# researchmm/MM-Diffusion

Hardware: AMD Instinct MI355X
Metric: denoising steps/sec (video+audio pair), 16x64x64 / 25600 (higher is better)
Workload: dtype bf16; 1 GPU; BASELINE configs[1]: Landscape base model (133.68M params), DDPM p_sample, timestep_respacing=250, per-GPU batch 4, 16x3x64x64 video + 1x25600 audio; global_batch=4, parallelism=batch-sharded x1, no in-loop collective, weights=key-seeded synthetic (mm_diffusion.synth), graph_replay=True, batch_lanes=2, finite=True, ranks_seen=1

## Files before the change

### include/mmd.h

```cpp
#ifndef MMD_H
#define MMD_H
#include <stdint.h>
#ifdef __cplusplus
extern "C" {
#endif

#define MMD_F32 0
#define MMD_BF16 1
#define MMD_OK 0
#define MMD_ERR_ARG (-1)
#define MMD_ERR_LAUNCH (-2)
#define MMD_ERR_UNSUPPORTED (-3)

int mmd_version(void);
const char* mmd_last_error(void);
int mmd_debug_install_crash_handler(void);

int mmd_graph_begin(void* stream);
int mmd_graph_end(void* stream, void** exec_out);
int mmd_graph_launch(void* exec, void* stream);
int mmd_graph_destroy(void* exec);
int mmd_stream_create(void** stream_out);
int mmd_stream_sync(void* stream);
int mmd_stream_destroy(void* stream);
// ... 65 lines not shown
int mmd_tattn_block(const void* X, int64_t ldx, const void* A, int64_t lda, void* MID, int64_t ldm, const void* Wf,
                    const float* bias_pre, const float* bias_qkv, const float* bias_proj, const float* gamma, const float* beta,
                    float eps, void* Y, int64_t ldy, int N, int F, int HW, int C, int heads, float* stats, int64_t stats_ld,
                    void* stream);

int64_t mmd_tconv_weight_bytes(int Cin, int Cout);
int mmd_tconv_pack(const void* W, void* out, int Cin, int Cout, void* stream);
int mmd_tconv(const void* X, int64_t ldx, const void* Wf, const float* bias, void* Y, int64_t ldy, int N, int F, int HW, int Cin,
              int Cout, float* stats, int64_t stats_ld, void* stream);

int mmd_aconv(const void* X, int64_t ldx, const void* W, const float* bias, const float* ga, const float* gb, int act, void* Y, int64_t ldy,
              int M, int L, int Cin, int Cout, int dil, float* stats, int64_t stats_ld, void* stream);

int mmd_attn_fwd(int dtype, const void* Q, int64_t ldq, int q_off, const void* KV, int64_t ldkv, int k_off, int v_off, void* O,
                 int64_t ldo, int heads, int ch, int nb, int G, int64_t q_rows_per_batch, int q_per_group,
                 int64_t k_rows_per_batch, int k_per_group, int win, const int* shift_dev, int impl, void* stream);
int mmd_attn_small_fwd(int dtype, const void* QKV, int64_t ld, void* O, int64_t ldo, int C, int heads, int S, int Tn, int inner,
                       int64_t outer_stride, int64_t inner_stride, int64_t tstride, void* stream);

int mmd_resample(int dtype, const void* x, int64_t ldx, void* y, int64_t ldy, int C, int NF, int H, int W, int fh, int fw,
                 int mode, float scale, void* stream);
int mmd_resample_stats(const void* x, int64_t ldx, void* y, int64_t ldy, int C, int NF, int H, int W, int fh, int fw, int mode,
                       float* stats, int64_t stats_ld, void* stream);
int mmd_copy2d(const void* x, int64_t ldx_bytes, void* y, int64_t ldy_bytes, int64_t rows, int64_t row_bytes, void* stream);

int mmd_stem_conv(int dtype, const float* x, const float* w, const float* bias, void* y, int64_t ldy, int N, int F, int Cin,
                  int H, int W, int Cout, int ntaps, const int* taps, void* stream);
int mmd_head_conv(int dtype, const void* x, int64_t ldx, const float* w, const float* bias, float* y, int N, int F, int Cin,
                  int H, int W, int Co, int ntaps, const int* taps, void* stream);
int64_t mmd_head_gemm_weight_bytes(int Cin);
int64_t mmd_head_gemm_workspace_bytes(int64_t M, int ntaps, int Co);
int mmd_head_gemm(const void* x, int64_t ldx, int64_t M, int Cin, const float* gn_a, const float* gn_b, int S, int64_t gn_rows, int act,
                  const void* wimg, float* P, int NO, void* stream);
int mmd_head_gather(const float* P, const float* bias, float* y, int N, int F, int H, int W, int Co, int ntaps, const int* taps,
                    void* stream);

int mmd_ddpm_update(const float* x, const float* model_out, const float* noise, float* out, float* x0_out, float* mean_out,
                    float* logvar_out, const float* tables, const int64_t* t, int T, int N, int F, int C, int HW, int flags,
                    void* stream);
int mmd_q_sample(const float* x0, const float* eps, float* out, const float* tab2, const int64_t* t, int T, int N,
                 int64_t per_sample, void* stream);

int64_t mmd_loss_workspace_bytes(int N);
int mmd_loss_terms(const float* x0, const float* xt, const float* model_out, const float* target, const float* tables,
                   const int64_t* t, int T, int N, int F, int C, int HW, int flags, float vb_scale, float* mse_out, float* vb_out,
                   void* workspace, void* stream);
// ... 104 lines not shown
```

### mm-diffusion_amd/csrc/mmd_misc.hip

```cpp
#include "mmd_common.h"

__global__ __launch_bounds__(256) void temb_kernel(const void* __restrict__ t, int t_kind, int dim, const float* __restrict__ W0,
                                                   const float* __restrict__ b0, const float* __restrict__ W2,
                                                   const float* __restrict__ b2, float* __restrict__ out_silu,
                                                   float* __restrict__ out_raw) {
  extern __shared__ float sm[];
  float* e = sm;
  float* h = sm + dim;
  const int n = blockIdx.x, tid = threadIdx.x;
  float tv;
  if (t_kind == 0) tv = (float)((const int64_t*)t)[n];
  else if (t_kind == 1) tv = (float)((const int32_t*)t)[n];
  else tv = ((const float*)t)[n];
  const int half = dim / 2;
  for (int i = tid; i < dim; i += 256) {
    float v = 0.f;
    if (i < 2 * half) {
      const int k = i < half ? i : i - half;
      const float f = expf(-logf(10000.f) * (float)k / (float)half);
      const float a = tv * f;
      v = i < half ? cosf(a) : sinf(a);
    }
    e[i] = v;
  }
  __syncthreads();
  for (int j = tid; j < dim; j += 256) {
    float a = b0[j];
    for (int k = 0; k < dim; ++k) a += W0[j * dim + k] * e[k];
    h[j] = silu_f(a);
  }
  __syncthreads();
  for (int j = tid; j < dim; j += 256) {
    float a = b2[j];
    for (int k = 0; k < dim; ++k) a += W2[j * dim + k] * h[k];
    if (out_raw) out_raw[n * dim + j] = a;
    out_silu[n * dim + j] = silu_f(a);
  }
}

__global__ __launch_bounds__(256) void linear_kernel(const float* __restrict__ x, const float* __restrict__ W,
                                                     const float* __restrict__ b, float* __restrict__ y, int N, int K, int J) {
  const int lane = threadIdx.x & 63;
  const int j = blockIdx.x * 4 + (threadIdx.x >> 6);
  if (j >= J) return;
  for (int n0 = 0; n0 < N; n0 += 8) {
    float acc[8];
#pragma unroll
    for (int i = 0; i < 8; ++i) acc[i] = 0.f;
    for (int k = lane; k < K; k += 64) {
      const float w = W[(int64_t)j * K + k];
#pragma unroll
      for (int i = 0; i < 8; ++i)
        if (n0 + i < N) acc[i] += w * x[(int64_t)(n0 + i) * K + k];
    }
#pragma unroll
    for (int i = 0; i < 8; ++i) {
      const float s = wave_sum(acc[i]);
      if (lane == 0 && n0 + i < N) y[(int64_t)(n0 + i) * J + j] = s + (b ? b[j] : 0.f);
    }
  }
}

template <typename T>
__global__ __launch_bounds__(256) void resample_kernel(const char* __restrict__ x, int64_t ldx, char* __restrict__ y, int64_t ldy,
                                                       int C, int NF, int H, int W, int fh, int fw, int mode, float scale) {
  constexpr int EPV = Elt<T>::EPV;
  constexpr int ES = 16 / EPV;
  const int CV = C / EPV;
  const int Ho = mode == 0 ? H / fh : H * fh, Wo = mode == 0 ? W / fw : W * fw;
  const int64_t total = (int64_t)NF * Ho * Wo * CV;
  for (int64_t i = (int64_t)blockIdx.x * 256 + threadIdx.x; i < total; i += (int64_t)gridDim.x * 256) {
    const int cv = (int)(i % CV);
    const int64_t orow = i / CV;
    const int wo = (int)(orow % Wo), ho = (int)((orow / Wo) % Ho);
    const int64_t nf = orow / ((int64_t)Wo * Ho);
    float acc[EPV];
    if (mode == 0) {
#pragma unroll
      for (int e = 0; e < EPV; ++e) acc[e] = 0.f;
      for (int a = 0; a < fh; ++a)
        for (int b = 0; b < fw; ++b) {
          const int64_t irow = (nf * H + ho * fh + a) * W + wo * fw + b;
          float f[EPV];
          Elt<T>::unpack(*(const u32x4*)(x + (irow * ldx + (int64_t)cv * EPV) * ES), f);
#pragma unroll
          for (int e = 0; e < EPV; ++e) acc[e] += f[e];
        }
      const float inv = scale / (float)(fh * fw);
#pragma unroll
      for (int e = 0; e < EPV; ++e) acc[e] *= inv;
      *(u32x4*)(y + (orow * ldy + (int64_t)cv * EPV) * ES) = Elt<T>::pack(acc);
    } else {
      const int64_t irow = (nf * H + ho / fh) * W + wo / fw;
      u32x4 v = *(const u32x4*)(x + (irow * ldx + (int64_t)cv * EPV) * ES);
      if (scale != 1.f) {
        Elt<T>::unpack(v, acc);
#pragma unroll
        for (int e = 0; e < EPV; ++e) acc[e] *= scale;
        v = Elt<T>::pack(acc);
      }
      *(u32x4*)(y + (orow * ldy + (int64_t)cv * EPV) * ES) = v;
    }
  }
}

__global__ __launch_bounds__(256) void resample_stats_kernel(const char* __restrict__ x, int64_t ldx, char* __restrict__ y, int64_t ldy, int C,
                                                             int NF, int H, int W, int fh, int fw, int mode, float* __restrict__ stats,
                                                             int64_t stats_ld, int nrec, int lcvp) {
  __shared__ float sPart[256 * 4];
  const int tid = threadIdx.x, CV = C >> 3;
  const int cv = tid & ((1 << lcvp) - 1), rg = tid >> lcvp, rgn = 256 >> lcvp;
  const int Ho = mode == 0 ? H / fh : H * fh, Wo = mode == 0 ? W / fw : W * fw;
  const float inv = 1.f / (float)(fh * fw);
  for (int rec = blockIdx.x; rec < nrec; rec += gridDim.x) {
    float s0 = 0.f, s1 = 0.f, q0 = 0.f, q1 = 0.f;
    if (cv < CV) {
#pragma unroll 4
      for (int r = rg; r < 64; r += rgn) {
        const int orow = rec * 64 + r;
        const int wo = orow % Wo, t = orow / Wo, ho = t % Ho, nf = t / Ho;
        u32x4 v;
        if (mode == 0) {
          float acc[8];
#pragma unroll
          for (int e = 0; e < 8; ++e) acc[e] = 0.f;
          for (int a = 0; a < fh; ++a)
            for (int b = 0; b < fw; ++b) {
              const int64_t irow = ((int64_t)nf * H + ho * fh + a) * W + wo * fw + b;
              float f[8];
              Elt<__bf16>::unpack(*(const u32x4*)(x + (irow * ldx + (int64_t)cv * 8) * 2), f);
#pragma unroll
              for (int e = 0; e < 8; ++e) acc[e] += f[e];
            }
#pragma unroll
          for (int e = 0; e < 8; ++e) acc[e] *= inv;
          v = Elt<__bf16>::pack(acc);
        } else {
          const int64_t irow = ((int64_t)nf * H + ho / fh) * W + wo / fw;
          v = *(const u32x4*)(x + (irow * ldx + (int64_t)cv * 8) * 2);
        }
        *(u32x4*)(y + ((int64_t)orow * ldy + (int64_t)cv * 8) * 2) = v;
        float f[8];
        Elt<__bf16>::unpack(v, f);
#pragma unroll
        for (int j = 0; j < 4; ++j) {
          s0 += f[j];
          s1 += f[4 + j];
          q0 += f[j] * f[j];
          q1 += f[4 + j] * f[4 + j];
        }
      }
    }
    *(f32x4*)(sPart + tid * 4) = f32x4{s0, s1, q0, q1};
    __syncthreads();
    if (rg == 0 && cv < CV) {
      for (int g = 1; g < rgn; ++g) {
        const f32x4 o = *(const f32x4*)(sPart + ((g << lcvp) + cv) * 4);
        s0 += o[0];
        s1 += o[1];
        q0 += o[2];
        q1 += o[3];
      }
      *(f32x4*)(stats + ((int64_t)rec * stats_ld + 2 * cv) * 2) = f32x4{s0, q0, s1, q1};
    }
    __syncthreads();
  }
}

__global__ __launch_bounds__(256) void copy2d_kernel(const char* __restrict__ x, int64_t ldx_b, char* __restrict__ y, int64_t ldy_b,
                                                     int64_t rows, int vecs) {
  const int64_t total = rows * vecs;
  for (int64_t i = (int64_t)blockIdx.x * 256 + threadIdx.x; i < total; i += (int64_t)gridDim.x * 256) {
    const int64_t r = i / vecs;
    const int v = (int)(i % vecs);
    *(u32x4*)(y + r * ldy_b + (int64_t)v * 16) = *(const u32x4*)(x + r * ldx_b + (int64_t)v * 16);
  }
}

extern "C" int mmd_temb_fwd(const void* t, int t_kind, int N, int dim, const float* W0, const float* b0, const float* W2,
                            const float* b2, float* out_silu, float* out_raw, void* stream) {
  MMD_REQUIRE(t && W0 && b0 && W2 && b2 && out_silu && N > 0 && dim > 0 && dim <= 4096, "temb_fwd: bad argument");
  MMD_REQUIRE(t_kind >= 0 && t_kind <= 2, "temb_fwd: t_kind must be 0 (int64), 1 (int32) or 2 (float32)");
  return mmd_launch<temb_kernel>("temb", dim3(N), dim3(256), 2 * dim * sizeof(float), (hipStream_t)stream, t, t_kind, dim, W0, b0, W2, b2, out_silu, out_raw);
}

extern "C" int mmd_linear_fwd(const float* x, const float* W, const float* b, float* y, int N, int K, int J, void* stream) {
  MMD_REQUIRE(x && W && y && N > 0 && K > 0 && J > 0, "linear_fwd: bad argument");
  return mmd_launch<linear_kernel>("linear", dim3(cdiv(J, 4)), dim3(256), 0, (hipStream_t)stream, x, W, b, y, N, K, J);
}
// ... 6 lines not shown
  MMD_REQUIRE(mode == 1 || (H % fh == 0 && W % fw == 0), "resample: pooled dims must divide (%d/%d, %d/%d)", H, fh, W, fw);
  const int64_t orows = mode == 0 ? (int64_t)NF * (H / fh) * (W / fw) : (int64_t)NF * H * fh * W * fw;
  const int grid = ew_grid(orows * (C / epv));
  hipStream_t st = (hipStream_t)stream;
  return mmd_by_dtype(dtype, [&](auto t) {
    return mmd_launch<resample_kernel<typename decltype(t)::type>>("resample", dim3(grid), dim3(256), 0, st, (const char*)x, ldx, (char*)y, ldy, C, NF, H, W,
                                                                   fh, fw, mode, scale);
  });
}

extern "C" int mmd_resample_stats(const void* x, int64_t ldx, void* y, int64_t ldy, int C, int NF, int H, int W, int fh, int fw, int mode,
                                  float* stats, int64_t stats_ld, void* stream) {
  MMD_REQUIRE(x && y && stats && C > 0 && C % 8 == 0 && C <= 2048 && NF > 0 && H > 0 && W > 0 && fh > 0 && fw > 0 && (mode == 0 || mode == 1),
              "resample_stats: bad argument (bf16 rows of 8 .. 2048 channels in whole 16-byte vectors)");
  MMD_REQUIRE(mode == 1 || (H % fh == 0 && W % fw == 0), "resample_stats: pooled dims must divide (%d/%d, %d/%d)", H, fh, W, fw);
  const int64_t orows = mode == 0 ? (int64_t)NF * (H / fh) * (W / fw) : (int64_t)NF * H * fh * W * fw;
  MMD_REQUIRE(orows % 64 == 0 && orows < ((int64_t)1 << 31), "resample_stats: %ld output rows (records are 64 rows; < 2^31)", (long)orows);
  MMD_REQUIRE((uintptr_t)stats % 16 == 0 && stats_ld % 2 == 0 && stats_ld >= C / 4, "resample_stats: the record view must start on an even quad "
              "of a 16-byte aligned buffer (ld %ld quads)", (long)stats_ld);
  MMD_REQUIRE(((uintptr_t)x | (uintptr_t)y) % 16 == 0 && ldx % 8 == 0 && ldy % 8 == 0, "resample_stats: unaligned rows");
  int lcvp = 0;
  while ((1 << lcvp) < C / 8) ++lcvp;
  const int nrec = (int)(orows / 64);
  return mmd_launch<resample_stats_kernel>("resample_stats", dim3(min(nrec, 8192)), dim3(256), 0, (hipStream_t)stream, (const char*)x, ldx, (char*)y, ldy, C,
                                           NF, H, W, fh, fw, mode, stats, stats_ld, nrec, lcvp);
}

extern "C" int mmd_copy2d(const void* x, int64_t ldx_bytes, void* y, int64_t ldy_bytes, int64_t rows, int64_t row_bytes, void* stream) {
  MMD_REQUIRE(x && y && rows > 0 && row_bytes > 0 && row_bytes % 16 == 0 && ldx_bytes % 16 == 0 && ldy_bytes % 16 == 0,
              "copy2d: rows must be 16-byte multiples");
  MMD_REQUIRE(((uintptr_t)x | (uintptr_t)y) % 16 == 0, "copy2d: unaligned pointer");
  const int vecs = (int)(row_bytes / 16);
  return mmd_launch<copy2d_kernel>("copy2d", dim3(ew_grid(rows * vecs)), dim3(256), 0, (hipStream_t)stream, (const char*)x, ldx_bytes, (char*)y, ldy_bytes,
                                   rows, vecs);
}

__global__ void timestep_embedding_kernel(const void* __restrict__ t, int t_kind, int dim, float* __restrict__ out) {
  const int n = blockIdx.x;
  float tv;
  if (t_kind == 0) tv = (float)((const int64_t*)t)[n];
  else if (t_kind == 1) tv = (float)((const int32_t*)t)[n];
  else tv = ((const float*)t)[n];
  const int half = dim / 2;
  for (int i = threadIdx.x; i < dim; i += blockDim.x) {
    float v = 0.f;
    if (i < 2 * half) {
      const int k = i < half ? i : i - half;
      const float a = tv * expf(-logf(10000.f) * (float)k / (float)half);
// ... 24 lines not shown
```

### mm-diffusion_amd/csrc/mmd_norm.hip

```cpp
#include "mmd_common.h"

#define GN_GROUPS 32
typedef __attribute__((ext_vector_type(2))) double f64x2;

struct SliceGeom {
  int S, Tn, inner;
  int64_t outer_stride, inner_stride, tstride;
};

__device__ __forceinline__ int64_t slice_base(const SliceGeom& g, int s) {
  return (int64_t)(s / g.inner) * g.outer_stride + (int64_t)(s % g.inner) * g.inner_stride;
}
__device__ __forceinline__ int slice_of_row(const SliceGeom& g, int64_t m) {
  const int64_t o = m / g.outer_stride, rem = m % g.outer_stride;
  return (int)(o * g.inner + (rem / g.inner_stride) % g.inner);
}

template <typename T, bool ONE>
__global__ __launch_bounds__(256) void gn_partial_kernel(const char* __restrict__ x, int64_t ld, int C, SliceGeom g, int R,
                                                         double* __restrict__ part, int nchunks,
                                                         const float* __restrict__ gamma, const float* __restrict__ beta,
                                                         const float* __restrict__ film, int64_t film_ld, float eps,
                                                         float* __restrict__ a_out, float* __restrict__ b_out, float* __restrict__ mr_out) {
  constexpr int EPV = Elt<T>::EPV;
// ... 221 lines not shown
        for (int e = 0; e < EPV; ++e) {
          const float w = f[e] * av[e] + bv[e];
          f[e] = act ? silu_f(w) : w;
        }
        *(u32x4*)(yp + (int64_t)j * ys) = Elt<T>::pack(f);
      }
    }
  }
  }
}

template <typename T>
__global__ __launch_bounds__(256) void gn_small_kernel(const char* __restrict__ x, int64_t ldx, char* __restrict__ y, int64_t ldy, int C,
                                                       SliceGeom g, const float* __restrict__ gamma, const float* __restrict__ beta,
                                                       float eps, int act, int SPB) {
  constexpr int EPV = Elt<T>::EPV, ES = 16 / EPV, MAXT = 16, QPV = EPV / 4;
  extern __shared__ __attribute__((aligned(16))) char smem[];
  float* sQ = (float*)smem;
  const int CV = C / EPV, NQ = C / 4, cpg = C / GN_GROUPS, qpg = cpg / 4;
  const int tid = threadIdx.x, pl = tid / CV, cv = tid - pl * CV;
  const int s = blockIdx.x * SPB + pl;
  const bool live = pl < SPB && s < g.S;
  u32x4 v[MAXT];
  const int64_t base = live ? slice_base(g, s) : 0;
  const char* xp = x + (base * ldx + (int64_t)cv * EPV) * ES;
  const int64_t xs = g.tstride * ldx * ES;
#pragma unroll
  for (int j = 0; j < MAXT; ++j)
    if (live && j < g.Tn) v[j] = *(const u32x4*)(xp + (int64_t)j * xs);
  float q[2] = {0.f, 0.f};
  if (live) {
#pragma unroll
    for (int j = 0; j < MAXT; ++j)
      if (j < g.Tn) {
        float f[EPV];
        Elt<T>::unpack(v[j], f);
#pragma unroll
        for (int e = 0; e < EPV; ++e) q[e / 4] += f[e];
      }
#pragma unroll
    for (int h = 0; h < QPV; ++h) sQ[pl * NQ + cv * QPV + h] = q[h];
  }
  __syncthreads();
  const float inv_cnt = 1.f / ((float)cpg * (float)g.Tn);
  float mean[2] = {0.f, 0.f};
  if (live) {
#pragma unroll
    for (int h = 0; h < QPV; ++h) {
      const int gi = (cv * QPV + h) / qpg;
      float a = 0.f;
      for (int k = 0; k < qpg; ++k) a += sQ[pl * NQ + gi * qpg + k];
      mean[h] = a * inv_cnt;
// ... 4 lines not shown
    q[0] = q[1] = 0.f;
#pragma unroll
    for (int j = 0; j < MAXT; ++j)
      if (j < g.Tn) {
        float f[EPV];
        Elt<T>::unpack(v[j], f);
#pragma unroll
        for (int e = 0; e < EPV; ++e) { const float d = f[e] - mean[e / 4]; q[e / 4] += d * d; }
      }
#pragma unroll
    for (int h = 0; h < QPV; ++h) sQ[pl * NQ + cv * QPV + h] = q[h];
  }
  __syncthreads();
  if (live) {
    float av[EPV], bv[EPV];
#pragma unroll
    for (int h = 0; h < QPV; ++h) {
      const int gi = (cv * QPV + h) / qpg;
      float a = 0.f;
      for (int k = 0; k < qpg; ++k) a += sQ[pl * NQ + gi * qpg + k];
      const float rstd = rsqrtf(a * inv_cnt + eps);
#pragma unroll
      for (int e = 0; e < 4; ++e) {
        const int c = cv * EPV + h * 4 + e;
        av[h * 4 + e] = rstd * gamma[c];
        bv[h * 4 + e] = beta[c] - mean[h] * av[h * 4 + e];
      }
    }
    char* yp = y + (base * ldy + (int64_t)cv * EPV) * ES;
    const int64_t ys = g.tstride * ldy * ES;
#pragma unroll
    for (int j = 0; j < MAXT; ++j)
      if (j < g.Tn) {
        float f[EPV];
        Elt<T>::unpack(v[j], f);
#pragma unroll
        for (int e = 0; e < EPV; ++e) {
          const float w = f[e] * av[e] + bv[e];
          f[e] = act ? silu_f(w) : w;
        }
        *(u32x4*)(yp + (int64_t)j * ys) = Elt<T>::pack(f);
      }
  }
}

template <typename T>
__global__ __launch_bounds__(256) void add_rowbias_kernel(char* __restrict__ x, int64_t ld, int64_t rows, int C,
                                                          int64_t rows_per_sample, const float* __restrict__ e, int64_t e_ld) {
  constexpr int EPV = Elt<T>::EPV;
// ... 270 lines not shown
extern "C" int mmd_add_rowbias(int dtype, void* x, int64_t ld, int64_t rows, int C, int64_t rows_per_sample, const float* e,
                               int64_t e_ld, void* stream) {
  MMD_REQUIRE(dtype == MMD_BF16 || dtype == MMD_F32, "add_rowbias: bad dtype");
  MMD_REQUIRE(x && e && rows > 0 && C % 8 == 0, "add_rowbias: bad argument");
  const int64_t total = rows * (C / (dtype == MMD_BF16 ? 8 : 4));
  const int grid = (int)min((int64_t)4096, (total + 255) / 256);
  hipStream_t st = (hipStream_t)stream;
  return mmd_by_dtype(dtype, [&](auto t) {
    return mmd_launch<add_rowbias_kernel<typename decltype(t)::type>>("add_rowbias", dim3(grid), dim3(256), 0, st, (char*)x, ld, rows, C, rows_per_sample, e, e_ld);
  });
}

extern "C" int mmd_gn_small(int dtype, const void* x, int64_t ldx, void* y, int64_t ldy, int C, int S, int Tn, int inner,
                            int64_t outer_stride, int64_t inner_stride, int64_t tstride, const float* gamma, const float* beta,
                            float eps, int act, void* stream) {
  int rc = check_geom("gn_small", dtype, C, S, Tn, inner);
  if (rc) return rc;
  MMD_REQUIRE(C / (dtype == MMD_BF16 ? 8 : 4) <= 256, "gn_small: rows of at most 256 16-byte vectors (C = %d)", C);
  MMD_REQUIRE(x && y && gamma && beta, "gn_small: null pointer");
  MMD_REQUIRE(Tn <= 16 && (C / GN_GROUPS) % 4 == 0, "gn_small: slices of at most 16 rows, groups of whole channel quads (got Tn=%d C=%d)", Tn, C);
  SliceGeom g{S, Tn, inner, outer_stride, inner_stride, tstride};
  const int cv = C / (dtype == MMD_BF16 ? 8 : 4);
  MMD_REQUIRE(cv <= 256, "gn_small: %d channels is too wide", C);
  const int spb = 256 / cv;
  const size_t lds = (size_t)spb * (C / 4) * sizeof(float);
  return mmd_by_dtype(dtype, [&](auto t) {
    return mmd_launch<gn_small_kernel<typename decltype(t)::type>>("gn_small", dim3(cdiv(S, spb)), dim3(256), lds, (hipStream_t)stream, (const char*)x, ldx,
                                                                   (char*)y, ldy, C, g, gamma, beta, eps, act, spb);
  });
}
```

### mm-diffusion_amd/mm_diffusion/_hip.py

```python
import ctypes as C
import gc
import os

import torch

_HERE = os.path.dirname(os.path.abspath(__file__))
LIB_PATH = os.environ.get("MMD_LIB") or os.path.join(os.path.dirname(_HERE), "lib", "libmmd.so")

F32, BF16 = 0, 1
_lib = None

i32, i64, f32, vp = C.c_int, C.c_int64, C.c_float, C.c_void_p


_PROTOS = {
    "mmd_version": (C.c_int, []),
    "mmd_last_error": (C.c_char_p, []),
    "mmd_debug_install_crash_handler": (i32, []),
    "mmd_graph_begin": (i32, [vp]),
    "mmd_graph_end": (i32, [vp, C.POINTER(vp)]),
    "mmd_graph_launch": (i32, [vp, vp]),
    "mmd_graph_destroy": (i32, [vp]),
    "mmd_stream_create": (i32, [C.POINTER(vp)]),
    "mmd_stream_sync": (i32, [vp]),
# ... 14 lines not shown
    "mmd_colsum_slices": (i32, [i32, vp, i64, i32, i64, i32, vp, i64, vp]),
    "mmd_conv_gemm": (i32, [i32, vp, i64, vp, vp, vp, i64, vp, i64, i32, i32, i32, i32, C.POINTER(i32), i32, i32, i32, i32, vp]),
    "mmd_gn_conv1x1": (i32, [i32, vp, i64, vp, vp, i32, i32, i64, vp, vp, vp, i64, vp, i64, i32, i32, i32, i32, vp]),
    "mmd_conv_gemm_stats": (i32, [i32, vp, i64, vp, vp, vp, i64, vp, i64, i32, i32, i32, i32, C.POINTER(i32), i32, i32, i32, i32, vp, i64, vp]),
    "mmd_gn_conv1x1_stats": (i32, [i32, vp, i64, vp, vp, i32, i32, i64, vp, vp, vp, i64, vp, i64, i32, i32, i32, i32, vp, i64, vp]),
    "mmd_gn_conv1x1_skip": (i32, [i32, vp, i64, vp, vp, i32, i32, i64, vp, vp, vp, i64, i32, vp, vp, vp, i64, i32, i32, i32, vp, i64, vp]),
    "mmd_gn_conv_gemm": (i32, [i32, vp, i64, vp, vp, i32, i32, i64, vp, vp, vp, i64, vp, i64, i32, i32, i32, i32, C.POINTER(i32), i32, i32, i32, i32, vp]),
    "mmd_tconv_weight_bytes": (i64, [i32, i32]),
    "mmd_tconv_pack": (i32, [vp, vp, i32, i32, vp]),
    "mmd_tconv": (i32, [vp, i64, vp, vp, vp, i64, i32, i32, i32, i32, i32, vp, i64, vp]),
    "mmd_aconv": (i32, [vp, i64, vp, vp, vp, vp, i32, vp, i64, i32, i32, i32, i32, i32, vp, i64, vp]),
    "mmd_tattn_weight_bytes": (i64, [i32, i32]),
    "mmd_tattn_pack": (i32, [vp, vp, vp, vp, i32, vp]),
    "mmd_tattn_block": (i32, [vp, i64, vp, i64, vp, i64, vp, vp, vp, vp, vp, vp, f32, vp, i64, i32, i32, i32, i32, i32, vp, i64, vp]),
    "mmd_vconv2d1d_weight_bytes": (i64, [i32]),
    "mmd_vconv2d1d_pack": (i32, [vp, vp, vp, i32, i32, vp]),
    "mmd_vconv2d1d": (i32, [vp, i64, vp, vp, i32, i32, i64, vp, vp, vp, vp, i64, i32, i32, i32, i32, i32, i32, vp, i64, vp]),
    "mmd_zero": (i32, [vp, i64, vp]),
    "mmd_gn_finalize_stats": (i32, [vp, i64, i32, i32, i32, vp, vp, vp, i64, f32, vp, vp, vp, vp]),
    "mmd_attn_fwd": (i32, [i32, vp, i64, i32, vp, i64, i32, i32, vp, i64, i32, i32, i32, i32, i64, i32, i64, i32, i32, vp, i32, vp]),
    "mmd_attn_small_fwd": (i32, [i32, vp, i64, vp, i64, i32, i32, i32, i32, i32, i64, i64, i64, vp]),
    "mmd_resample": (i32, [i32, vp, i64, vp, i64, i32, i32, i32, i32, i32, i32, i32, f32, vp]),
    "mmd_resample_stats": (i32, [vp, i64, vp, i64, i32, i32, i32, i32, i32, i32, i32, vp, i64, vp]),
    "mmd_copy2d": (i32, [vp, i64, vp, i64, i64, i64, vp]),
    "mmd_stem_conv": (i32, [i32, vp, vp, vp, vp, i64, i32, i32, i32, i32, i32, i32, i32, C.POINTER(i32), vp]),
    "mmd_head_conv": (i32, [i32, vp, i64, vp, vp, vp, i32, i32, i32, i32, i32, i32, i32, C.POINTER(i32), vp]),
    "mmd_head_gemm_weight_bytes": (i64, [i32]),
    "mmd_head_gemm_workspace_bytes": (i64, [i64, i32, i32]),
    "mmd_head_gemm": (i32, [vp, i64, i64, i32, vp, vp, i32, i64, i32, vp, vp, i32, vp]),
    "mmd_head_gather": (i32, [vp, vp, vp, i32, i32, i32, i32, i32, i32, C.POINTER(i32), vp]),
    "mmd_ddpm_update": (i32, [vp, vp, vp, vp, vp, vp, vp, vp, vp, i32, i32, i32, i32, i32, i32, vp]),
    "mmd_loss_workspace_bytes": (i64, [i32]),
    "mmd_loss_terms": (i32, [vp, vp, vp, vp, vp, vp, i32, i32, i32, i32, i32, i32, f32, vp, vp, vp, vp]),
    "mmd_conv_wgrad": (i32, [i32, vp, i64, vp, i64, vp, vp, i32, i32, i32, i32, C.POINTER(i32), i32, i32, i32, i32, vp]),
    "mmd_gn_bwd": (i32, [i32, vp, i64, vp, i64, vp, i64, i64, i32, i32, i32, i32, i64, i64, i64, vp, vp, vp, vp, vp, vp, i64, i32, vp, vp, vp, i64, vp, vp]),
    "mmd_gn_bwd_ws0": (i32, [i32, vp, i64, vp, i64, vp, i64, i64, i32, i32, i32, i32, i64, i64, i64, vp, vp, vp, vp, vp, vp, i64, i32, vp, vp, vp, i64, vp, vp]),
    "mmd_attn_bwd": (i32, [i32, vp, i64, i32, vp, i64, i32, i32, vp, i64, vp, i64, vp, i64, i32, vp, i64, i32, i32, vp, vp, i32, i32, i32, i32,
                           i32, i64, i64, i64, i32, i32, i32, i64, i64, i64, i32, i32, i32, vp, vp]),
    "mmd_timestep_embedding": (i32, [vp, i32, i32, i32, vp, vp]),
    "mmd_attn_fwd_lse": (i32, [i32, vp, i64, i32, vp, i64, i32, i32, vp, i64, i32, i32, i32, i32, i64, i32, i64, i32, i32, vp, vp, vp]),
    "mmd_attn_bwd_mfma": (i32, [vp, i64, i32, vp, i64, i32, i32, vp, i64, vp, i64, vp, i64, i32, vp, i64, i32, i32, vp, vp, i32, i32, i32, i32,
                                i64, i32, i64, i32, i32, vp, vp]),
    "mmd_attn_small_bwd": (i32, [i32, vp, i64, vp, i64, vp, i64, i32, i32, i32, i32, i32, i64, i64, i64, vp]),
    "mmd_ddim_update": (i32, [vp, vp, vp, vp, vp, vp, vp, vp, i32, i32, i32, i32, i32, i32, f32, vp]),
    "mmd_lincomb_t": (i32, [vp, vp, vp, vp, vp, vp, vp, i32, i64, vp]),
    "mmd_lincomb": (i32, [vp, f32, vp, f32, vp, f32, vp, i64, vp]),
# ... 208 lines not shown
```

### mm-diffusion_amd/mm_diffusion/engine.py

```python
import os
from types import SimpleNamespace

import torch

from . import _hip as H
from . import ops
from .ops import Geom


_EMB_ON_AUDIO_STREAM = ops._flag("MMD_EMB_AUX")
_POOL_NOREUSE = os.environ.get("MMD_POOL_NOREUSE") == "1"
_UP_LOWRES = ops._flag("MMD_UP_LOWRES")
_CROSS_SERIAL = ops._flag("MMD_CROSS_SERIAL")
_RESAMPLE_STATS = ops._flag("MMD_RESAMPLE_STATS")
_SKIP_FUSE = ops._flag("MMD_SKIP_FUSE")


class _Pool:

    def __init__(self, device):
        self.device = device
        self.free = []
        self.all = []

    def get(self, nbytes):
        nbytes = (int(nbytes) + 255) // 256 * 256
        best = None
        for i, raw in enumerate(self.free):
            sz = raw.numel()
            if sz >= nbytes and sz <= 2 * nbytes + 65536 and (best is None or sz < self.free[best].numel()):
                best = i
        if best is not None:
            return self.free.pop(best)
        raw = torch.empty(nbytes, dtype=torch.uint8, device=self.device)
        self.all.append(raw)
        return raw

    def put(self, raw):
# ... 318 lines not shown
            self._release(ga, gb)
            return h
        t0 = self._gn(x, s.in_norm, s.gin, act=True)
        h = self._alloc(s.rows_in, s.cout, stats=s.hstats, unit=s.rows_in // N)
        ops.conv_gemm(t0, self._gemm_w(w), self._f32(b), taps=ops.taps_audio(dilation), dims=(L, 1, 1), out=h, **self._stats_kw(h))
        self._release(t0)
        return h

    def _res_out_low(self, s, x, h, out):
        ylow = self._res_tail(s, h, x, s.gin, s.film, lambda: self._alloc(s.rows_in, s.cout))
        self._release(h)
        dest = self._alloc(s.rows_out, s.cout, stats=True, unit=s.rows_out // self.N) if out is None else out
        ops.resample(ylow, dest, *s.rs, stats=self._resample_stats(dest))
        self._release(ylow)
        return dest

    def _res_out(self, s, x, h, out):
        if s.low_out:
            return self._res_out_low(s, x, h, out)
        per = s.rows_out // self.N
        xs = x
        if s.resampled:
            hp, xp = self._alloc(s.rows_out, s.cout, stats=s.ss, unit=per), self._alloc(s.rows_out, s.cin)
            ops.resample(h, hp, *s.rs, stats=self._resample_stats(hp))
            ops.resample(x, xp, *s.rs)
            self._release(h)
            h, xs = hp, xp
        if not s.ss:
            ops.add_rowbias(h, s.film, per)
        dest = self._res_tail(s, h, xs, Geom.per_sample(self.N, per), s.film if s.ss else None,
                              lambda: self._alloc(s.rows_out, s.cout, stats=True, unit=s.Ho * s.Ho if (s.attn and s.vid) else per)
                              if (s.attn or out is None) else out)
        self._release(h)
        if xs is not x:
            self._release(xs)
        return self._res_attn(s, dest, out) if s.attn else dest

    def _res_fin(self, s, out):
        return out if out is not None else self._alloc(s.rows_out, s.cout, stats=True, unit=s.rows_out // self.N)

    def _res_attn(self, s, dest, out):
        p, Ho = s.p, s.Ho
        if not s.vid:
            fin = self._res_fin(s, out)
            self._self_attn(dest, p + ".audio_attention_block", "audio", Ho, fin)
            self._release(dest)
        elif self._tattn_fused and ops.tattn_pre_ok(dest, self.model.num_heads, self.N, self.F, Ho * Ho):
            att = self._self_attn(dest, p + ".spatial_attention_block", "spatial", Ho, None, no_proj=True)
# ... 273 lines not shown
```

### mm-diffusion_amd/mm_diffusion/ops.py

```python
import contextlib
import os

import torch

from . import _hip as H

GN_EPS = 1e-5

_recorder = None
_keep = None


class recording:
    def __init__(self, plan, keep=None):
        self.plan, self.keep = plan, keep

    def __enter__(self):
        global _recorder, _keep
        self._prev, _recorder = (_recorder, _keep), self.plan
        _keep = self.keep
        return self.plan

    def __exit__(self, *a):
        global _recorder, _keep
# ... 716 lines not shown
def attn_small_bwd(qkv, dout, dqkv, C, heads, geom: Geom):
    _chk2d(qkv), _chk2d(dout), _chk2d(dqkv)
    _dispatch("mmd_attn_small_bwd", H.dt_of(qkv), qkv.data_ptr(), qkv.stride(0), dout.data_ptr(), dout.stride(0), dqkv.data_ptr(),
              dqkv.stride(0), C, heads, *geom.args(),
              meta=("attn_small_bwd", 10 * geom.S * geom.Tn * geom.Tn * C, 8 * geom.S * geom.Tn * C * qkv.element_size()))
    return dqkv


def resample(x, out, NF, Hh, Ww, fh, fw, mode, scale=1.0, stats=None):
    _chk2d(x), _chk2d(out)
    nbytes = (x.shape[0] + out.shape[0]) * x.shape[1] * x.element_size()
    if stats is not None:
        if x.dtype != torch.bfloat16 or out.dtype != torch.bfloat16 or float(scale) != 1.0:
            raise H.MMDError("resample: output statistics need bf16 rows and scale 1")
        sp, sld = _stats_args(stats, out.shape[0], x.shape[1])
        _dispatch("mmd_resample_stats", x.data_ptr(), x.stride(0), out.data_ptr(), out.stride(0), x.shape[1], NF, Hh, Ww, fh, fw, mode, sp, sld,
                  meta=("resample", 0, nbytes))
        return out
    _dispatch("mmd_resample", H.dt_of(x), x.data_ptr(), x.stride(0), out.data_ptr(), out.stride(0), x.shape[1], NF, Hh, Ww,
           fh, fw, mode, float(scale), meta=("resample", 0, nbytes))
    return out


def copy2d(x, out):
    _chk2d(x), _chk2d(out)
    es = x.element_size()
    _dispatch("mmd_copy2d", x.data_ptr(), x.stride(0) * es, out.data_ptr(), out.stride(0) * es, x.shape[0], x.shape[1] * es)
    return out


def _t_kind(t):
    kind = {torch.int64: 0, torch.int32: 1, torch.float32: 2}.get(t.dtype)
    if kind is None:
        raise H.MMDError(f"timesteps must be int64/int32/float32, got {t.dtype}")
    return kind


def temb(t, dim, W0, b0, W2, b2, out_silu, out_raw=None):
    kind = _t_kind(t)
    H.require_cuda(t, W0)
    _dispatch("mmd_temb_fwd", t.data_ptr(), kind, t.shape[0], dim, W0.data_ptr(), b0.data_ptr(), W2.data_ptr(), b2.data_ptr(),
           out_silu.data_ptr(), H.ptr(out_raw))
    return out_silu


def linear(x, W, b, out):
# ... 399 lines not shown
```

Baseline: 367.6 pair-steps/s.

## Fuse paired resamples, specialize 2x2 pooling, unroll linear kernel, tune gn_small

Adds a pair kernel that resamples the residual branch with group-norm statistics and the skip input in one launch, gated behind an opt-in flag. Resample kernels get a specialized 2x2 pooling path that batches independent loads, plus 32-bit indexing when it fits. The linear kernel is templated on row count with 8-way unrolled loads, and gn_small now preloads gamma/beta, loads unconditionally, and picks a smaller slices-per-block and thread count to raise block count. The changes aim to cut launch count and memory latency across small bandwidth-bound kernels, at the cost of more template variants and register pressure.

```diff
diff --git a/include/mmd.h b/include/mmd.h
--- a/include/mmd.h
+++ b/include/mmd.h
@@ -111,6 +111,8 @@
                  int mode, float scale, void* stream);
 int mmd_resample_stats(const void* x, int64_t ldx, void* y, int64_t ldy, int C, int NF, int H, int W, int fh, int fw, int mode,
                        float* stats, int64_t stats_ld, void* stream);
+int mmd_resample_pair(const void* h, int64_t ldh, void* hp, int64_t ldhp, int Ch, float* stats, int64_t stats_ld, const void* x,
+                      int64_t ldx, void* xp, int64_t ldxp, int Cx, int NF, int H, int W, int fh, int fw, int mode, void* stream);
 int mmd_copy2d(const void* x, int64_t ldx_bytes, void* y, int64_t ldy_bytes, int64_t rows, int64_t row_bytes, void* stream);
 
 int mmd_stem_conv(int dtype, const float* x, const float* w, const float* bias, void* y, int64_t ldy, int N, int F, int Cin,
diff --git a/mm-diffusion_amd/csrc/mmd_misc.hip b/mm-diffusion_amd/csrc/mmd_misc.hip
--- a/mm-diffusion_amd/csrc/mmd_misc.hip
+++ b/mm-diffusion_amd/csrc/mmd_misc.hip
@@ -38,83 +38,179 @@
   }
 }
 
+template <int NI>
+__device__ __forceinline__ void linear_rows(const float* __restrict__ x, const float* __restrict__ Wj, float bj, float* __restrict__ y, int n0,
+                                            int K, int J, int j, int lane) {
+  float acc[NI];
+#pragma unroll
+  for (int i = 0; i < NI; ++i) acc[i] = 0.f;
+  for (int k0 = lane; k0 < K; k0 += 512) {
+    float w[8], xv[8][NI];
+#pragma unroll
+    for (int u = 0; u < 8; ++u) {
+      const int kc = min(k0 + 64 * u, K - 1);
+      w[u] = Wj[kc];
+#pragma unroll
+      for (int i = 0; i < NI; ++i) xv[u][i] = x[(int64_t)(n0 + i) * K + kc];
+    }
+#pragma unroll
+    for (int u = 0; u < 8; ++u)
+      if (k0 + 64 * u < K) {
+#pragma unroll
+        for (int i = 0; i < NI; ++i) acc[i] += w[u] * xv[u][i];
+      }
+  }
+#pragma unroll
+  for (int i = 0; i < NI; ++i) {
+    const float s = wave_sum(acc[i]);
+    if (lane == 0) y[(int64_t)(n0 + i) * J + j] = s + bj;
+  }
+}
+
 __global__ __launch_bounds__(256) void linear_kernel(const float* __restrict__ x, const float* __restrict__ W,
                                                      const float* __restrict__ b, float* __restrict__ y, int N, int K, int J) {
   const int lane = threadIdx.x & 63;
   const int j = blockIdx.x * 4 + (threadIdx.x >> 6);
   if (j >= J) return;
+  const float* Wj = W + (int64_t)j * K;
+  const float bj = b ? b[j] : 0.f;
   for (int n0 = 0; n0 < N; n0 += 8) {
-    float acc[8];
-#pragma unroll
-    for (int i = 0; i < 8; ++i) acc[i] = 0.f;
-    for (int k = lane; k < K; k += 64) {
-      const float w = W[(int64_t)j * K + k];
-#pragma unroll
-      for (int i = 0; i < 8; ++i)
-        if (n0 + i < N) acc[i] += w * x[(int64_t)(n0 + i) * K + k];
-    }
-#pragma unroll
-    for (int i = 0; i < 8; ++i) {
-      const float s = wave_sum(acc[i]);
-      if (lane == 0 && n0 + i < N) y[(int64_t)(n0 + i) * J + j] = s + (b ? b[j] : 0.f);
-    }
+    switch (min(N - n0, 8)) {
+      case 1: linear_rows<1>(x, Wj, bj, y, n0, K, J, j, lane); break;
+      case 2: linear_rows<2>(x, Wj, bj, y, n0, K, J, j, lane); break;
+      case 3: linear_rows<3>(x, Wj, bj, y, n0, K, J, j, lane); break;
+      case 4: linear_rows<4>(x, Wj, bj, y, n0, K, J, j, lane); break;
+      case 5: linear_rows<5>(x, Wj, bj, y, n0, K, J, j, lane); break;
+      case 6: linear_rows<6>(x, Wj, bj, y, n0, K, J, j, lane); break;
+      case 7: linear_rows<7>(x, Wj, bj, y, n0, K, J, j, lane); break;
+      default: linear_rows<8>(x, Wj, bj, y, n0, K, J, j, lane); break;
+    }
+  }
+}
+
+template <typename T, int NT, typename IX>
+__device__ __forceinline__ void resample_span(const char* __restrict__ x, int64_t ldx, char* __restrict__ y, int64_t ldy, int C, int H, int W,
+                                              int fh, int fw, int mode, float scale, IX first, IX step, IX total) {
+  constexpr int EPV = Elt<T>::EPV;
+  constexpr int ES = 16 / EPV;
+  const IX CV = C / EPV;
+  const IX Ho = mode == 0 ? H / fh : H * fh, Wo = mode == 0 ? W / fw : W * fw;
+  const float inv = scale / (float)(fh * fw);
+  if constexpr (NT == 0) {
+    for (IX i = first; i < total; i += step) {
+      const int cv = (int)(i % CV);
+      const int64_t orow = i / CV;
+      const int wo = (int)(orow % Wo), ho = (int)((orow / Wo) % Ho);
+      const int64_t nf = orow / ((int64_t)Wo * Ho);
+      float acc[EPV];
+      if (mode == 0) {
+#pragma unroll
+        for (int e = 0; e < EPV; ++e) acc[e] = 0.f;
+        for (int a = 0; a < fh; ++a)
+          for (int b = 0; b < fw; ++b) {
+            const int64_t irow = (nf * H + ho * fh + a) * W + wo * fw + b;
+            float f[EPV];
+            Elt<T>::unpack(*(const u32x4*)(x + (irow * ldx + (int64_t)cv * EPV) * ES), f);
+#pragma unroll
+            for (int e = 0; e < EPV; ++e) acc[e] += f[e];
+          }
+#pragma unroll
+        for (int e = 0; e < EPV; ++e) acc[e] *= inv;
+        *(u32x4*)(y + (orow * ldy + (int64_t)cv * EPV) * ES) = Elt<T>::pack(acc);
+      } else {
+        const int64_t irow = (nf * H + ho / fh) * W + wo / fw;
+        u32x4 v = *(const u32x4*)(x + (irow * ldx + (int64_t)cv * EPV) * ES);
+        if (scale != 1.f) {
+          Elt<T>::unpack(v, acc);
+#pragma unroll
+          for (int e = 0; e < EPV; ++e) acc[e] *= scale;
+          v = Elt<T>::pack(acc);
+        }
+        *(u32x4*)(y + (orow * ldy + (int64_t)cv * EPV) * ES) = v;
+      }
+    }
+  } else {
+    constexpr int NR = 2;
+    int64_t toff[NT];
+#pragma unroll
+    for (int t = 0; t < NT; ++t) toff[t] = ((int64_t)(t / fw) * W + t % fw) * ldx * ES;
+    for (IX i0 = first; i0 < total; i0 += NR * step) {
+      u32x4 v[NR][NT];
+      int64_t yo[NR];
+#pragma unroll
+      for (int u = 0; u < NR; ++u) {
+        const IX i = i0 + u * step < total ? i0 + u * step : total - 1;
+        const IX cv = i % CV, orow = i / CV;
+        const IX wo = orow % Wo, t = orow / Wo, ho = t % Ho, nf = t / Ho;
+        const char* p = x + ((((int64_t)nf * H + ho * fh) * W + wo * fw) * ldx + (int64_t)cv * EPV) * ES;
+#pragma unroll
+        for (int k = 0; k < NT; ++k) v[u][k] = *(const u32x4*)(p + toff[k]);
+        yo[u] = ((int64_t)orow * ldy + (int64_t)cv * EPV) * ES;
+      }
+#pragma unroll
+      for (int u = 0; u < NR; ++u)
+        if (u == 0 || i0 + u * step < total) {
+          float acc[EPV];
+#pragma unroll
+          for (int e = 0; e < EPV; ++e) acc[e] = 0.f;
+#pragma unroll
+          for (int k = 0; k < NT; ++k) {
+            float f[EPV];
+            Elt<T>::unpack(v[u][k], f);
+#pragma unroll
+            for (int e = 0; e < EPV; ++e) acc[e] += f[e];
+          }
+#pragma unroll
+          for (int e = 0; e < EPV; ++e) acc[e] *= inv;
+          *(u32x4*)(y + yo[u]) = Elt<T>::pack(acc);
+        }
+    }
+  }
+}
+
+template <typename T>
+__device__ __forceinline__ void resample_blocks(const char* __restrict__ x, int64_t ldx, char* __restrict__ y, int64_t ldy, int C, int NF, int H,
+                                                int W, int fh, int fw, int mode, float scale, int blk, int nb) {
+  const int Ho = mode == 0 ? H / fh : H * fh, Wo = mode == 0 ? W / fw : W * fw;
+  const int64_t total = (int64_t)NF * Ho * Wo * (C / Elt<T>::EPV), first = (int64_t)blk * 256 + threadIdx.x, step = (int64_t)nb * 256;
+  const bool four = mode == 0 && fh * fw == 4;
+  if (total + 2 * step < ((int64_t)1 << 31)) {
+    if (four) resample_span<T, 4, int>(x, ldx, y, ldy, C, H, W, fh, fw, mode, scale, (int)first, (int)step, (int)total);
+    else resample_span<T, 0, int>(x, ldx, y, ldy, C, H, W, fh, fw, mode, scale, (int)first, (int)step, (int)total);
+  } else {
+    if (four) resample_span<T, 4, int64_t>(x, ldx, y, ldy, C, H, W, fh, fw, mode, scale, first, step, total);
+    else resample_span<T, 0, int64_t>(x, ldx, y, ldy, C, H, W, fh, fw, mode, scale, first, step, total);
   }
 }
 
 template <typename T>
 __global__ __launch_bounds__(256) void resample_kernel(const char* __restrict__ x, int64_t ldx, char* __restrict__ y, int64_t ldy,
                                                        int C, int NF, int H, int W, int fh, int fw, int mode, float scale) {
-  constexpr int EPV = Elt<T>::EPV;
-  constexpr int ES = 16 / EPV;
-  const int CV = C / EPV;
-  const int Ho = mode == 0 ? H / fh : H * fh, Wo = mode == 0 ? W / fw : W * fw;
-  const int64_t total = (int64_t)NF * Ho * Wo * CV;
-  for (int64_t i = (int64_t)blockIdx.x * 256 + threadIdx.x; i < total; i += (int64_t)gridDim.x * 256) {
-    const int cv = (int)(i % CV);
-    const int64_t orow = i / CV;
-    const int wo = (int)(orow % Wo), ho = (int)((orow / Wo) % Ho);
-    const int64_t nf = orow / ((int64_t)Wo * Ho);
-    float acc[EPV];
-    if (mode == 0) {
-#pragma unroll
-      for (int e = 0; e < EPV; ++e) acc[e] = 0.f;
-      for (int a = 0; a < fh; ++a)
-        for (int b = 0; b < fw; ++b) {
-          const int64_t irow = (nf * H + ho * fh + a) * W + wo * fw + b;
-          float f[EPV];
-          Elt<T>::unpack(*(const u32x4*)(x + (irow * ldx + (int64_t)cv * EPV) * ES), f);
-#pragma unroll
-          for (int e = 0; e < EPV; ++e) acc[e] += f[e];
-        }
-      const float inv = scale / (float)(fh * fw);
-#pragma unroll
-      for (int e = 0; e < EPV; ++e) acc[e] *= inv;
-      *(u32x4*)(y + (orow * ldy + (int64_t)cv * EPV) * ES) = Elt<T>::pack(acc);
-    } else {
-      const int64_t irow = (nf * H + ho / fh) * W + wo / fw;
-      u32x4 v = *(const u32x4*)(x + (irow * ldx + (int64_t)cv * EPV) * ES);
-      if (scale != 1.f) {
-        Elt<T>::unpack(v, acc);
-#pragma unroll
-        for (int e = 0; e < EPV; ++e) acc[e] *= scale;
-        v = Elt<T>::pack(acc);
-      }
-      *(u32x4*)(y + (orow * ldy + (int64_t)cv * EPV) * ES) = v;
-    }
-  }
-}
-
-__global__ __launch_bounds__(256) void resample_stats_kernel(const char* __restrict__ x, int64_t ldx, char* __restrict__ y, int64_t ldy, int C,
-                                                             int NF, int H, int W, int fh, int fw, int mode, float* __restrict__ stats,
-                                                             int64_t stats_ld, int nrec, int lcvp) {
-  __shared__ float sPart[256 * 4];
+  resample_blocks<T>(x, ldx, y, ldy, C, NF, H, W, fh, fw, mode, scale, blockIdx.x, gridDim.x);
+}
+
+template <int NT>
+__device__ __forceinline__ void resample_record(const char* __restrict__ x, int64_t ldx, char* __restrict__ y, int64_t ldy, int C, int H, int W,
+                                                int fh, int fw, int mode, float* __restrict__ stats, int64_t stats_ld, int rec, int lcvp,
+                                                float* sPart) {
   const int tid = threadIdx.x, CV = C >> 3;
   const int cv = tid & ((1 << lcvp) - 1), rg = tid >> lcvp, rgn = 256 >> lcvp;
   const int Ho = mode == 0 ? H / fh : H * fh, Wo = mode == 0 ? W / fw : W * fw;
   const float inv = 1.f / (float)(fh * fw);
-  for (int rec = blockIdx.x; rec < nrec; rec += gridDim.x) {
-    float s0 = 0.f, s1 = 0.f, q0 = 0.f, q1 = 0.f;
-    if (cv < CV) {
+  float s0 = 0.f, s1 = 0.f, q0 = 0.f, q1 = 0.f;
+  auto fold = [&](const u32x4& v) {
+    float f[8];
+    Elt<__bf16>::unpack(v, f);
+#pragma unroll
+    for (int j = 0; j < 4; ++j) {
+      s0 += f[j];
+      s1 += f[4 + j];
+      q0 += f[j] * f[j];
+      q1 += f[4 + j] * f[4 + j];
+    }
+  };
+  if (cv < CV) {
+    if constexpr (NT == 0) {
 #pragma unroll 4
       for (int r = rg; r < 64; r += rgn) {
         const int orow = rec * 64 + r;
@@ -140,31 +236,82 @@
           v = *(const u32x4*)(x + (irow * ldx + (int64_t)cv * 8) * 2);
         }
         *(u32x4*)(y + ((int64_t)orow * ldy + (int64_t)cv * 8) * 2) = v;
-        float f[8];
-        Elt<__bf16>::unpack(v, f);
-#pragma unroll
-        for (int j = 0; j < 4; ++j) {
-          s0 += f[j];
-          s1 += f[4 + j];
-          q0 += f[j] * f[j];
-          q1 += f[4 + j] * f[4 + j];
+        fold(v);
+      }
+    } else if (rg < 64) {
+      constexpr int NR = 4;
+      int64_t toff[NT];
+#pragma unroll
+      for (int t = 0; t < NT; ++t) toff[t] = ((int64_t)(t / fw) * W + t % fw) * ldx * 2;
+      for (int r0 = rg; r0 < 64; r0 += NR * rgn) {
+        u32x4 v[NR][NT];
+        int64_t yo[NR];
+#pragma unroll
+        for (int u = 0; u < NR; ++u) {
+          const int r = r0 + u * rgn < 64 ? r0 + u * rgn : r0;
+          const int orow = rec * 64 + r;
+          const int wo = orow % Wo, t = orow / Wo, ho = t % Ho, nf = t / Ho;
+          const char* p = x + ((((int64_t)nf * H + ho * fh) * W + wo * fw) * ldx + (int64_t)cv * 8) * 2;
+#pragma unroll
+          for (int k = 0; k < NT; ++k) v[u][k] = *(const u32x4*)(p + toff[k]);
+          yo[u] = ((int64_t)orow * ldy + (int64_t)cv * 8) * 2;
         }
+#pragma unroll
+        for (int u = 0; u < NR; ++u)
+          if (u == 0 || r0 + u * rgn < 64) {
+            float acc[8];
+#pragma unroll
+            for (int e = 0; e < 8; ++e) acc[e] = 0.f;
+#pragma unroll
+            for (int k = 0; k < NT; ++k) {
+              float f[8];
+              Elt<__bf16>::unpack(v[u][k], f);
+#pragma unroll
+              for (int e = 0; e < 8; ++e) acc[e] += f[e];
+            }
+#pragma unroll
+            for (int e = 0; e < 8; ++e) acc[e] *= inv;
+            const u32x4 o = Elt<__bf16>::pack(acc);
+            *(u32x4*)(y + yo[u]) = o;
+            fold(o);
+          }
       }
     }
-    *(f32x4*)(sPart + tid * 4) = f32x4{s0, s1, q0, q1};
-    __syncthreads();
-    if (rg == 0 && cv < CV) {
-      for (int g = 1; g < rgn; ++g) {
-        const f32x4 o = *(const f32x4*)(sPart + ((g << lcvp) + cv) * 4);
-        s0 += o[0];
-        s1 += o[1];
-        q0 += o[2];
-        q1 += o[3];
-      }
-      *(f32x4*)(stats + ((int64_t)rec * stats_ld + 2 * cv) * 2) = f32x4{s0, q0, s1, q1};
-    }
-    __syncthreads();
-  }
+  }
+  *(f32x4*)(sPart + tid * 4) = f32x4{s0, s1, q0, q1};
+  __syncthreads();
+  if (rg == 0 && cv < CV) {
+    for (int g = 1; g < rgn; ++g) {
+      const f32x4 o = *(const f32x4*)(sPart + ((g << lcvp) + cv) * 4);
+      s0 += o[0];
+      s1 += o[1];
+      q0 += o[2];
+      q1 += o[3];
+    }
+    *(f32x4*)(stats + ((int64_t)rec * stats_ld + 2 * cv) * 2) = f32x4{s0, q0, s1, q1};
+  }
+  __syncthreads();
+}
+
+template <int NT>
+__global__ __launch_bounds__(256) void resample_stats_kernel(const char* __restrict__ x, int64_t ldx, char* __restrict__ y, int64_t ldy, int C,
+                                                             int NF, int H, int W, int fh, int fw, int mode, float* __restrict__ stats,
+                                                             int64_t stats_ld, int nrec, int lcvp) {
+  __shared__ float sPart[256 * 4];
+  for (int rec = blockIdx.x; rec < nrec; rec += gridDim.x)
+    resample_record<NT>(x, ldx, y, ldy, C, H, W, fh, fw, mode, stats, stats_ld, rec, lcvp, sPart);
+}
+
+template <int NT>
+__global__ __launch_bounds__(256) void resample_pair_kernel(const char* __restrict__ h, int64_t ldh, char* __restrict__ hp, int64_t ldhp, int Ch,
+                                                            float* __restrict__ stats, int64_t stats_ld, int nrec, int lcvp,
+                                                            const char* __restrict__ x, int64_t ldx, char* __restrict__ xp, int64_t ldxp, int Cx,
+                                                            int NF, int H, int W, int fh, int fw, int mode) {
+  __shared__ float sPart[256 * 4];
+  if ((int)blockIdx.x < nrec)
+    resample_record<NT>(h, ldh, hp, ldhp, Ch, H, W, fh, fw, mode, stats, stats_ld, blockIdx.x, lcvp, sPart);
+  else
+    resample_blocks<__bf16>(x, ldx, xp, ldxp, Cx, NF, H, W, fh, fw, mode, 1.f, blockIdx.x - nrec, gridDim.x - nrec);
 }
 
 __global__ __launch_bounds__(256) void copy2d_kernel(const char* __restrict__ x, int64_t ldx_b, char* __restrict__ y, int64_t ldy_b,
@@ -217,8 +364,33 @@
   int lcvp = 0;
   while ((1 << lcvp) < C / 8) ++lcvp;
   const int nrec = (int)(orows / 64);
-  return mmd_launch<resample_stats_kernel>("resample_stats", dim3(min(nrec, 8192)), dim3(256), 0, (hipStream_t)stream, (const char*)x, ldx, (char*)y, ldy, C,
-                                           NF, H, W, fh, fw, mode, stats, stats_ld, nrec, lcvp);
+  if (mode == 0 && fh * fw == 4)
+    return mmd_launch<resample_stats_kernel<4>>("resample_stats", dim3(min(nrec, 8192)), dim3(256), 0, (hipStream_t)stream, (const char*)x, ldx, (char*)y, ldy,
+                                                C, NF, H, W, fh, fw, mode, stats, stats_ld, nrec, lcvp);
+  return mmd_launch<resample_stats_kernel<0>>("resample_stats", dim3(min(nrec, 8192)), dim3(256), 0, (hipStream_t)stream, (const char*)x, ldx, (char*)y, ldy,
+                                              C, NF, H, W, fh, fw, mode, stats, stats_ld, nrec, lcvp);
+}
+
+extern "C" int mmd_resample_pair(const void* h, int64_t ldh, void* hp, int64_t ldhp, int Ch, float* stats, int64_t stats_ld, const void* x,
+                                 int64_t ldx, void* xp, int64_t ldxp, int Cx, int NF, int H, int W, int fh, int fw, int mode, void* stream) {
+  MMD_REQUIRE(h && hp && stats && x && xp && Ch > 0 && Ch % 8 == 0 && Ch <= 2048 && Cx > 0 && Cx % 8 == 0 && NF > 0 && H > 0 && W > 0 && fh > 0 &&
+              fw > 0 && (mode == 0 || mode == 1), "resample_pair: bad argument (bf16 rows in whole 16-byte vectors, h of 8 .. 2048 channels)");
+  MMD_REQUIRE(mode == 1 || (H % fh == 0 && W % fw == 0), "resample_pair: pooled dims must divide (%d/%d, %d/%d)", H, fh, W, fw);
+  const int64_t orows = mode == 0 ? (int64_t)NF * (H / fh) * (W / fw) : (int64_t)NF * H * fh * W * fw;
+  MMD_REQUIRE(orows % 64 == 0 && orows < ((int64_t)1 << 31), "resample_pair: %ld output rows (records are 64 rows; < 2^31)", (long)orows);
+  MMD_REQUIRE((uintptr_t)stats % 16 == 0 && stats_ld % 2 == 0 && stats_ld >= Ch / 4, "resample_pair: the record view must start on an even quad "
+              "of a 16-byte aligned buffer (ld %ld quads)", (long)stats_ld);
+  MMD_REQUIRE(((uintptr_t)h | (uintptr_t)hp | (uintptr_t)x | (uintptr_t)xp) % 16 == 0 && ldh % 8 == 0 && ldhp % 8 == 0 && ldx % 8 == 0 && ldxp % 8 == 0,
+              "resample_pair: unaligned rows");
+  int lcvp = 0;
+  while ((1 << lcvp) < Ch / 8) ++lcvp;
+  const int nrec = (int)(orows / 64);
+  const int nxb = ew_grid(orows * (Cx / 8));
+  if (mode == 0 && fh * fw == 4)
+    return mmd_launch<resample_pair_kernel<4>>("resample_pair", dim3(nrec + nxb), dim3(256), 0, (hipStream_t)stream, (const char*)h, ldh, (char*)hp, ldhp, Ch,
+                                               stats, stats_ld, nrec, lcvp, (const char*)x, ldx, (char*)xp, ldxp, Cx, NF, H, W, fh, fw, mode);
+  return mmd_launch<resample_pair_kernel<0>>("resample_pair", dim3(nrec + nxb), dim3(256), 0, (hipStream_t)stream, (const char*)h, ldh, (char*)hp, ldhp, Ch,
+                                             stats, stats_ld, nrec, lcvp, (const char*)x, ldx, (char*)xp, ldxp, Cx, NF, H, W, fh, fw, mode);
 }
 
 extern "C" int mmd_copy2d(const void* x, int64_t ldx_bytes, void* y, int64_t ldy_bytes, int64_t rows, int64_t row_bytes, void* stream) {
diff --git a/mm-diffusion_amd/csrc/mmd_norm.hip b/mm-diffusion_amd/csrc/mmd_norm.hip
--- a/mm-diffusion_amd/csrc/mmd_norm.hip
+++ b/mm-diffusion_amd/csrc/mmd_norm.hip
@@ -267,12 +267,17 @@
   const int s = blockIdx.x * SPB + pl;
   const bool live = pl < SPB && s < g.S;
   u32x4 v[MAXT];
-  const int64_t base = live ? slice_base(g, s) : 0;
+  const int64_t base = slice_base(g, live ? s : 0);
   const char* xp = x + (base * ldx + (int64_t)cv * EPV) * ES;
   const int64_t xs = g.tstride * ldx * ES;
 #pragma unroll
-  for (int j = 0; j < MAXT; ++j)
-    if (live && j < g.Tn) v[j] = *(const u32x4*)(xp + (int64_t)j * xs);
+  for (int j = 0; j < MAXT; ++j) v[j] = *(const u32x4*)(xp + (int64_t)min(j, g.Tn - 1) * xs);
+  float gm[EPV], bt[EPV];
+#pragma unroll
+  for (int e = 0; e < EPV; ++e) {
+    gm[e] = gamma[cv * EPV + e];
+    bt[e] = beta[cv * EPV + e];
+  }
   float q[2] = {0.f, 0.f};
   if (live) {
 #pragma unroll
@@ -323,9 +328,8 @@
       const float rstd = rsqrtf(a * inv_cnt + eps);
 #pragma unroll
       for (int e = 0; e < 4; ++e) {
-        const int c = cv * EPV + h * 4 + e;
-        av[h * 4 + e] = rstd * gamma[c];
-        bv[h * 4 + e] = beta[c] - mean[h] * av[h * 4 + e];
+        av[h * 4 + e] = rstd * gm[h * 4 + e];
+        bv[h * 4 + e] = bt[h * 4 + e] - mean[h] * av[h * 4 + e];
       }
     }
     char* yp = y + (base * ldy + (int64_t)cv * EPV) * ES;
@@ -642,10 +646,14 @@
   SliceGeom g{S, Tn, inner, outer_stride, inner_stride, tstride};
   const int cv = C / (dtype == MMD_BF16 ? 8 : 4);
   MMD_REQUIRE(cv <= 256, "gn_small: %d channels is too wide", C);
-  const int spb = 256 / cv;
+  int spb = 256 / cv;
+  for (int c = spb; c >= 1; --c)
+    if (c * cv % 64 == 0) { spb = c; break; }
+  while (spb % 2 == 0 && (spb / 2) * cv % 64 == 0 && cdiv(S, spb) < 256) spb /= 2;
   const size_t lds = (size_t)spb * (C / 4) * sizeof(float);
+  const int threads = (spb * cv + 63) / 64 * 64;
   return mmd_by_dtype(dtype, [&](auto t) {
-    return mmd_launch<gn_small_kernel<typename decltype(t)::type>>("gn_small", dim3(cdiv(S, spb)), dim3(256), lds, (hipStream_t)stream, (const char*)x, ldx,
+    return mmd_launch<gn_small_kernel<typename decltype(t)::type>>("gn_small", dim3(cdiv(S, spb)), dim3(threads), lds, (hipStream_t)stream, (const char*)x, ldx,
                                                                    (char*)y, ldy, C, g, gamma, beta, eps, act, spb);
   });
 }
diff --git a/mm-diffusion_amd/mm_diffusion/_hip.py b/mm-diffusion_amd/mm_diffusion/_hip.py
--- a/mm-diffusion_amd/mm_diffusion/_hip.py
+++ b/mm-diffusion_amd/mm_diffusion/_hip.py
@@ -60,6 +60,7 @@
     "mmd_attn_small_fwd": (i32, [i32, vp, i64, vp, i64, i32, i32, i32, i32, i32, i64, i64, i64, vp]),
     "mmd_resample": (i32, [i32, vp, i64, vp, i64, i32, i32, i32, i32, i32, i32, i32, f32, vp]),
     "mmd_resample_stats": (i32, [vp, i64, vp, i64, i32, i32, i32, i32, i32, i32, i32, vp, i64, vp]),
+    "mmd_resample_pair": (i32, [vp, i64, vp, i64, i32, vp, i64, vp, i64, vp, i64, i32, i32, i32, i32, i32, i32, i32, vp]),
     "mmd_copy2d": (i32, [vp, i64, vp, i64, i64, i64, vp]),
     "mmd_stem_conv": (i32, [i32, vp, vp, vp, vp, i64, i32, i32, i32, i32, i32, i32, i32, C.POINTER(i32), vp]),
     "mmd_head_conv": (i32, [i32, vp, i64, vp, vp, vp, i32, i32, i32, i32, i32, i32, i32, C.POINTER(i32), vp]),
diff --git a/mm-diffusion_amd/mm_diffusion/engine.py b/mm-diffusion_amd/mm_diffusion/engine.py
--- a/mm-diffusion_amd/mm_diffusion/engine.py
+++ b/mm-diffusion_amd/mm_diffusion/engine.py
@@ -14,6 +14,7 @@
 _CROSS_SERIAL = ops._flag("MMD_CROSS_SERIAL")
 _RESAMPLE_STATS = ops._flag("MMD_RESAMPLE_STATS")
 _SKIP_FUSE = ops._flag("MMD_SKIP_FUSE")
+_RESAMPLE_PAIR = ops._flag("MMD_RESAMPLE_PAIR")
 
 
 class _Pool:
@@ -378,8 +379,12 @@
         xs = x
         if s.resampled:
             hp, xp = self._alloc(s.rows_out, s.cout, stats=s.ss, unit=per), self._alloc(s.rows_out, s.cin)
-            ops.resample(h, hp, *s.rs, stats=self._resample_stats(hp))
-            ops.resample(x, xp, *s.rs)
+            rec = self._resample_stats(hp)
+            if _RESAMPLE_PAIR and rec is not None and x.dtype == h.dtype == torch.bfloat16:
+                ops.resample_pair(h, hp, rec, x, xp, *s.rs)
+            else:
+                ops.resample(h, hp, *s.rs, stats=rec)
+                ops.resample(x, xp, *s.rs)
             self._release(h)
             h, xs = hp, xp
         if not s.ss:
diff --git a/mm-diffusion_amd/mm_diffusion/ops.py b/mm-diffusion_amd/mm_diffusion/ops.py
--- a/mm-diffusion_amd/mm_diffusion/ops.py
+++ b/mm-diffusion_amd/mm_diffusion/ops.py
@@ -762,6 +762,18 @@
     return out
 
 
+def resample_pair(h, hp, stats, x, xp, NF, Hh, Ww, fh, fw, mode):
+    for t in (h, hp, x, xp):
+        _chk2d(t)
+        if t.dtype != torch.bfloat16:
+            raise H.MMDError("resample_pair: bf16 rows only")
+    sp, sld = _stats_args(stats, hp.shape[0], h.shape[1])
+    nbytes = ((h.shape[0] + hp.shape[0]) * h.shape[1] + (x.shape[0] + xp.shape[0]) * x.shape[1]) * 2
+    _dispatch("mmd_resample_pair", h.data_ptr(), h.stride(0), hp.data_ptr(), hp.stride(0), h.shape[1], sp, sld, x.data_ptr(), x.stride(0),
+              xp.data_ptr(), xp.stride(0), x.shape[1], NF, Hh, Ww, fh, fw, mode, meta=("resample", 0, nbytes))
+    return hp, xp
+
+
 def copy2d(x, out):
     _chk2d(x), _chk2d(out)
     es = x.element_size()
```

After: 368.1 pair-steps/s (median of 2 runs). Within noise of the previous version (+0.1%).
